# ox-vgg/wise

Hardware: AMD Instinct MI355X
Metric: frames/sec embedded (ViT-B/32 bs=256) + queries/sec over 10M×512 index, 1/2/4/8 MI355X (higher is better)
Workload: dtype bf16; 1 GPU; OpenCLIP ViT-B/32 image tower (encode_image + L2 normalise), bs=256 frames per GPU, fp32 normalised frames resident in HBM -> [256,512] fp32 unit vectors; seeded random weights (no checkpoints offline); batches_in_flight=2, distinct_input_batches=4, layernorm_fold=True, global_batch=256, frames_per_gpu=256, parallelism=dp1, device=AMD Radeon Graphics

## Files before the change

wise_amd/csrc/gemm_bf16.hip:

```cpp
#include <utility>
#include <vector>

#include "common.h"
#include "transformer.h"
#include "gemm_shared.h"
#include "gemm_w4.h"

namespace wise {

struct GemmPlan {
    int splitk = 0;
    int n = 1;
    int v[2] = {0, 0};
    int rows[2] = {0, 0};
};

enum ConvTile { CONV_128x64 = 0, CONV_128x128 = 1, CONV_256x64 = 2, CONV_PP256 = 3 };

static int resolve_variant(int v, int M, int N, int K, int mode) {
    if (v >= 60 && v <= 70) {
        bool ok = false;
        switch (v) {
            case 60: ok = w4_shape_ok(M, N, K, 8); break;
            case 61: ok = w4_shape_ok(M, N, K, 5); break;
// ... 1754 lines not shown
static void launch_fold_consumer(int v, const bf16_t* A, const bf16_t* Wt, const float* bias, int M, int N, int K, bf16_t* out,
                                 const FoldArgs& fa, hipStream_t st) {
    switch (v) {
        case 60: launch_w4<MODE, 8, 8, 3, 2, 1, 1>(A, Wt, bias, M, N, K, out, st, fa); break;
        case 61: launch_w4<MODE, 5, 8, 3, 2, 1, 1>(A, Wt, bias, M, N, K, out, st, fa); break;
        case 64: launch_w4p<MODE, 1>(A, Wt, bias, M, N, K, out, device_cus(), st, fa); break;
        case 68: launch_w4<MODE, 4, 8, 3, 2, 1, 1>(A, Wt, bias, M, N, K, out, st, fa); break;
        case 66: launch_w4<MODE, 8, 6, 3, 2, 1, 1>(A, Wt, bias, M, N, K, out, st, fa); break;
        case 67: launch_w4<MODE, 4, 6, 3, 2, 1, 1>(A, Wt, bias, M, N, K, out, st, fa); break;
        case 69: launch_w4<MODE, 4, 6, 2, 2, 2, 1>(A, Wt, bias, M, N, K, out, st, fa); break;
        default: launch_w4<MODE, 4, 4, 3, 2, 2, 1>(A, Wt, bias, M, N, K, out, st, fa); break;
    }
}

int gemm_fold_bf16(const bf16_t* A, const bf16_t* Wt, const float* bias, const float* rstd, int M, int N, int K, int mode,
                   bf16_t* out, hipStream_t st) {
    WISE_CHECK_ARG(A && Wt && bias && rstd && out, "gemm_fold_bf16: null pointer");
    WISE_CHECK_ARG(gemm_fold_shape_ok(M, N, K) && bf16_out(mode) && mode != EPI_RELU, "gemm_fold_bf16: M=%d N=%d K=%d mode=%d", M, N, K, mode);
    ProfScope prof(PROF_GEMM, 2.0 * (double)M * (double)N * (double)K, st);
    FoldArgs fa;
    fa.stats = const_cast<float*>(rstd);
    const int v = fold_plan(M, N, K, mode, false, false, device_cus());
    WISE_CHECK_ARG(v != 0, "gemm_fold_bf16: no tile for M=%d N=%d K=%d", M, N, K);
    switch (mode) {
        case EPI_BF16: launch_fold_consumer<EPI_BF16>(v, A, Wt, bias, M, N, K, out, fa, st); break;
        case EPI_QUICKGELU: launch_fold_consumer<EPI_QUICKGELU>(v, A, Wt, bias, M, N, K, out, fa, st); break;
        case EPI_GELU: launch_fold_consumer<EPI_GELU>(v, A, Wt, bias, M, N, K, out, fa, st); break;
        default: launch_fold_consumer<EPI_GELU_TANH>(v, A, Wt, bias, M, N, K, out, fa, st); break;
    }
    WISE_LAUNCH_CHECK("gemm_w4_kernel (fold, bf16 out)");
    return WISE_OK;
}

size_t gemm_fold_stats_bytes(int M, int N) { return fold_stats_bytes(M, N); }
size_t gemm_fold_counters_bytes(int M) { return fold_count_slots(M) * 4; }

// ... 133 lines not shown
        const int r[6] = {p.splitk, p.n, p.v[0], p.rows[0], p.v[1], p.rows[1]};
        for (int i = 0; i < 6; ++i) out[i] = r[i];
        return 6;
    }
    if (kind == 1) {
        out[0] = wise::fold_plan(a[0], a[1], a[2], a[3], a[4] != 0, a[5] != 0, a[6]);
        return 1;
    }
    if (kind == 2) {
        out[0] = wise::conv_plan(wise::conv_rows(a[0], a[1], a[2], a[5] != 0), a[4]);
        return 1;
    }
    return 0;
}

extern "C" size_t wise_debug_gemm_splitk_bytes(int M, int m_valid, int N, int K) { return wise::gemm_splitk_bytes(M, m_valid, N, K); }
extern "C" int wise_debug_gemm_rows(const uint16_t* A, const uint16_t* Wt, const float* bias, int M, int m_valid, int N, int K,
                                    int mode, void* out, float* sk, size_t sk_bytes, void* stream) {
    return wise::gemm_bf16_rows(A, Wt, bias, M, m_valid, N, K, mode, out, (hipStream_t)stream, sk, sk_bytes);
}
extern "C" int wise_debug_gemm_resid_ln_rows(const uint16_t* A, const uint16_t* Wt, const float* bias, int M, int m_valid,
                                             int ln_rows, int N, int K, float* x, const float* ln_w, const float* ln_b, float eps,
                                             int post_ln, uint16_t* h, float* sk, size_t sk_bytes, void* stream) {
    return wise::gemm_resid_ln_rows(A, Wt, bias, M, m_valid, ln_rows, N, K, x, ln_w, ln_b, eps, post_ln != 0, h,
                                    (hipStream_t)stream, sk, sk_bytes);
}
#endif
```

wise_amd/csrc/gemm_w4.h:

```cpp
#pragma once
#include <type_traits>
#include "gemm_shared.h"

namespace wise {

struct FoldArgs {
    float* stats = nullptr;
    bf16_t* hcopy = nullptr;
    float eps = 1e-5f;
    int group32 = 0;
    int lo_off = 0;
};
__host__ __device__ inline size_t fold_count_slots(int M) { return (size_t)((M / 128 + 1 + 63) / 64 * 64); }
__host__ __device__ inline size_t fold_stats_bytes(int M, int N) { return (size_t)M * 4 + fold_count_slots(M) * 4 + (size_t)M * (N / 32) * 8; }

namespace w4 {

#ifdef W4_STAMPS
__device__ unsigned long long g_w4p_stamps[4][4];
#define W4P_STAMP(t, k) do { if (threadIdx.x == 0 && blockIdx.x == 0 && (t) < 4) g_w4p_stamps[t][k] = __builtin_amdgcn_s_memtime(); } while (0)
__device__ unsigned long long g_w4_stamps[2][4];
#define W4_STAMP(k)                                                                                              \
    do {                                                                                                         \
        if (threadIdx.x == 0 && (blockIdx.x == 0 || blockIdx.x == gridDim.x - 1))                                \
            g_w4_stamps[blockIdx.x == 0 ? 0 : 1][k] = __builtin_amdgcn_s_memtime();                              \
    } while (0)
// ... 131 lines not shown
        case 21: asm volatile("v_accvgpr_read_b32 %0, a244\n\tv_accvgpr_read_b32 %1, a245\n\tv_accvgpr_read_b32 %2, a246\n\tv_accvgpr_read_b32 %3, a247" : "=v"(r.x), "=v"(r.y), "=v"(r.z), "=v"(r.w) : : W4_HI_AGPRS); break;
        case 22: asm volatile("v_accvgpr_read_b32 %0, a248\n\tv_accvgpr_read_b32 %1, a249\n\tv_accvgpr_read_b32 %2, a250\n\tv_accvgpr_read_b32 %3, a251" : "=v"(r.x), "=v"(r.y), "=v"(r.z), "=v"(r.w) : : W4_HI_AGPRS); break;
        case 23: asm volatile("v_accvgpr_read_b32 %0, a252\n\tv_accvgpr_read_b32 %1, a253\n\tv_accvgpr_read_b32 %2, a254\n\tv_accvgpr_read_b32 %3, a255" : "=v"(r.x), "=v"(r.y), "=v"(r.z), "=v"(r.w) : : W4_HI_AGPRS); break;
        default: break;
    }
    return r;
}

template <int CTRL>
__device__ __forceinline__ float dpp_add(float v) {
    return v + __builtin_bit_cast(float, __builtin_amdgcn_update_dpp(0, __builtin_bit_cast(int, v), CTRL, 0xF, 0xF, true));
}

template <int MODE, int MI, int NJ, int RI, int FOLD = 0>
__device__ __forceinline__ void epi_bf16_pass(const f32x4 (&acc)[MI][NJ], int i0, const float4 (&bv)[NJ], bf16_t* __restrict__ out,
                                              int N, int row0, int col0, int lane, unsigned my,
                                              const float* __restrict__ rstd = nullptr) {
    constexpr int RS = NJ * 32 + 16, CPR = NJ * 2;
    static_assert((RI * 16 * CPR) % 64 == 0, "walk covers the piece in whole wave instructions");
    const int l15 = lane & 15, g = lane >> 4;
    float rs[RI];
    if constexpr (FOLD == 1) {
#pragma unroll
        for (int ii = 0; ii < RI; ++ii) rs[ii] = rstd[row0 + (i0 + ii) * 16 + l15];
    }
#pragma unroll
    for (int j = 0; j < NJ; j += 2)
#pragma unroll
        for (int ii = 0; ii < RI; ++ii) {
            const f32x4 a = acc[i0 + ii][j], b = acc[i0 + ii][j + 1];
            float x[8];
// ... 5 lines not shown
                x[0] = a[0] + bv[j].x; x[1] = a[1] + bv[j].y; x[2] = a[2] + bv[j].z; x[3] = a[3] + bv[j].w;
                x[4] = b[0] + bv[j + 1].x; x[5] = b[1] + bv[j + 1].y; x[6] = b[2] + bv[j + 1].z; x[7] = b[3] + bv[j + 1].w;
            }
            act_apply_n<MODE, 8>(x);
            W4_LDS(u32x2_t, my + (ii * 16 + l15) * RS + (j * 16 + g * 4) * 2) = u32x2_t{pack_bf16x2(x[0], x[1]), pack_bf16x2(x[2], x[3])};
            W4_LDS(u32x2_t, my + (ii * 16 + l15) * RS + ((j + 1) * 16 + g * 4) * 2) = u32x2_t{pack_bf16x2(x[4], x[5]), pack_bf16x2(x[6], x[7])};
        }
    __builtin_amdgcn_fence(__ATOMIC_RELEASE, "wavefront");
    __builtin_amdgcn_wave_barrier();
    __builtin_amdgcn_fence(__ATOMIC_ACQUIRE, "wavefront");
#pragma unroll
    for (int t = 0; t < RI * 16 * CPR / 64; ++t) {
        const int idx = t * 64 + lane, row = idx / CPR, c = idx % CPR;
        const u32x4_t v = W4_LDS(const u32x4_t, my + row * RS + c * 16);
#ifdef W4_PLAIN_STORES
        *reinterpret_cast<u32x4_t*>(out + (size_t)(row0 + i0 * 16 + row) * N + col0 + c * 8) = v;
#else
        __builtin_nontemporal_store(v, reinterpret_cast<u32x4_t*>(out + (size_t)(row0 + i0 * 16 + row) * N + col0 + c * 8));
#endif
    }
    __builtin_amdgcn_fence(__ATOMIC_RELEASE, "wavefront");
    __builtin_amdgcn_wave_barrier();
    __builtin_amdgcn_fence(__ATOMIC_ACQUIRE, "wavefront");
}

template <int NJ, int RI>
__device__ __forceinline__ void resid_load(const float* __restrict__ out, int N, int row0, int col0, int lane,
                                           float4 (&res)[RI * 16 * NJ * 4 / 64]) {
    constexpr int CPR = NJ * 4;
#pragma unroll
    for (int t = 0; t < RI * 16 * CPR / 64; ++t) {
        const int idx = t * 64 + lane, row = idx / CPR, c = idx % CPR;
        res[t] = *reinterpret_cast<const float4*>(out + (size_t)(row0 + row) * N + col0 + c * 4);
// ... 242 lines not shown
    mfma_retire();
#pragma unroll
    for (int m = 0; m < MI * NJ; ++m) { if (m < 64) pin_a(acc[m / NJ][m % NJ]); else pin_v(acc[m / NJ][m % NJ]); }

    W4_STAMP(2);
    asm volatile("s_waitcnt lgkmcnt(0)" ::: "memory");
    __builtin_amdgcn_s_barrier();
    const int row0 = m0 + wm * MI * 16, col0 = n0 + wn * NJ * 16;
    float4 bv[NJ];
#pragma unroll
    for (int j = 0; j < NJ; ++j)
        bv[j] = bias ? *reinterpret_cast<const float4*>(bias + col0 + j * 16 + g * 4) : make_float4(0.f, 0.f, 0.f, 0.f);
    const unsigned my = wave * 20480;
    if constexpr (bf16_out(MODE)) {
        bf16_t* o = reinterpret_cast<bf16_t*>(out);
        if constexpr (MI % 4 != 0) epi_bf16_pass<MODE, MI, NJ, MI % 4, FOLD>(acc, MI - MI % 4, bv, o, N, row0, col0, lane, my, fold.stats);
#pragma unroll
        for (int i0 = (MI / 4 - 1) * 4; i0 >= 0; i0 -= 4) epi_bf16_pass<MODE, MI, NJ, 4, FOLD>(acc, i0, bv, o, N, row0, col0, lane, my, fold.stats);
    } else {
        float* o = reinterpret_cast<float*>(out);
        constexpr int RP = NJ == 8 ? 2 : 1;
        constexpr int NP = (MI + RP - 1) / RP, NRES = RP * 16 * NJ * 4 / 64;
        static_assert(MI % RP == 0 || RP == 2, "passes");
        float4 res[2][NRES];
        auto load = [&](int p, float4 (&r)[NRES]) {
            if (p * RP + RP <= MI) {
                if constexpr (FOLD == 2) resid_load_hilo<NJ, RP>(fold.hcopy, fold.lo_off, N, row0 + p * RP * 16, col0, lane, r);
                else resid_load<NJ, RP>(o, N, row0 + p * RP * 16, col0, lane, r);
            } else if constexpr (RP == 2) {
                float4 (&h)[NRES / 2] = reinterpret_cast<float4 (&)[NRES / 2]>(r);
                if constexpr (FOLD == 2) resid_load_hilo<NJ, 1>(fold.hcopy, fold.lo_off, N, row0 + p * RP * 16, col0, lane, h);
                else resid_load<NJ, 1>(o, N, row0 + p * RP * 16, col0, lane, h);
            }
// ... 129 lines not shown

    f32x4 acc[MI][NJ];
    bf16x8 af0[MI], wf0[NJ], af1[MI], wf1[NJ];
    {
        lds_cptr pw = (lds_cptr)(uintptr_t)fw0, pa = (lds_cptr)(uintptr_t)fa0;
#pragma unroll
        for (int j = 0; j < NJ; ++j) wf0[j] = *reinterpret_cast<const __attribute__((address_space(3))) bf16x8*>(pw + j * 2048);
#pragma unroll
        for (int i = 0; i < MI; ++i) af0[i] = *reinterpret_cast<const __attribute__((address_space(3))) bf16x8*>(pa + i * 2048);
    }
    unsigned oA0 = 0, oA1 = ASZ, oA2 = 2 * ASZ;
    unsigned oW0 = 0, oW1 = WSZ, oW2 = 0;

    u32x2_t packed[MI][NJ];
    const __amdgpu_buffer_rsrc_t rO = __builtin_amdgcn_make_buffer_rsrc((void*)out, 0, 0x7fffffff, 0x00020000);
    const int vst = (g * N + l15 * 8) * 2;
    int sst = 0;
    typedef __attribute__((address_space(3))) unsigned char* lds_ptr;
    const lds_ptr scw = (lds_ptr)(uintptr_t)(scr + l15 * 272 + g * 8);
    const lds_cptr scrd = (lds_cptr)(uintptr_t)(scr + g * 272 + l15 * 16);
    auto load_bias = [&](int ncol, f32x4 (&b)[NJ]) {
#pragma unroll
        for (int j = 0; j < NJ; ++j) {
            const float4 v = bias ? *reinterpret_cast<const float4*>(bias + ncol + wn * 128 + j * 16 + g * 4) : make_float4(0.f, 0.f, 0.f, 0.f);
            b[j] = f32x4{v.x, v.y, v.z, v.w};
        }
    };
    f32x4 bv[NJ];
    float rs[MI];

    auto phase = [&](const bf16x8 (&af)[MI], const bf16x8 (&wf)[NJ], bf16x8 (&afn)[MI], bf16x8 (&wfn)[NJ], lds_cptr pw,
// ... 9 lines not shown
        for (int m = 0; m < NM; ++m) {
            if (m % MPR == 0 && m / MPR < NR) {
                const int r = m / MPR;
                if (r < NJ) wfn[r] = *reinterpret_cast<const __attribute__((address_space(3))) bf16x8*>(pw + r * 2048);
                else afn[r - NJ] = *reinterpret_cast<const __attribute__((address_space(3))) bf16x8*>(pa + (r - NJ) * 2048);
            }
            if (m >= 1 && (m - 1) % MPD == 0 && (m - 1) / MPD < ND) {
                const int u = ((m - 1) / MPD) * 4 + wave;
                dma16(rq, dslot + u * 1024, voff, u * 8 * ldb + dkb);
            }
            if (DW && m % 4 == 3 && m / 4 < NJ)
                *reinterpret_cast<__attribute__((address_space(3))) u32x2_t*>(scw + (m / 4) * 32) = packed[DI][m / 4];
            if (DR && m % 8 == 3 && m / 8 < 4)
                piece[m / 8] = *reinterpret_cast<const __attribute__((address_space(3))) u32x4_t*>(scrd + (m / 8) * 4 * 272);
            if (DR && m % 8 == 1 && m >= 9)
                __builtin_amdgcn_raw_buffer_store_b128(piece[m / 8 - 1], rO, vst, sst + (DI * 16 + (m / 8 - 1) * 4) * N * 2, 2);
            if (INIT) mfma16a_init(acc[m / NJ][m % NJ], wf[m % NJ], af[m / NJ]);
            else mfma16a(acc[m / NJ][m % NJ], wf[m % NJ], af[m / NJ]);
        }
    };

    auto step = [&](auto init_c, auto di_c, __amdgpu_buffer_rsrc_t rqA, __amdgpu_buffer_rsrc_t rqW, int kq) {
        constexpr int DI = decltype(di_c)::value;
        using DIc = std::integral_constant<int, DI < 0 ? 0 : DI>;
        using DOc = std::integral_constant<bool, (DI >= 0)>;
        phase(af0, wf0, af1, wf1, (lds_cptr)(uintptr_t)(oW0 + fw1), (lds_cptr)(uintptr_t)(oA0 + fa1), init_c,
              std::integral_constant<int, PA>{}, rqA, oA2, kq, DIc{}, DOc{}, std::false_type{});
        asm volatile("s_waitcnt lgkmcnt(0)" ::: "memory");
        wait_vmcnt<PA>();
        __builtin_amdgcn_s_barrier();
        phase(af1, wf1, af0, wf0, (lds_cptr)(uintptr_t)(oW1 + fw0), (lds_cptr)(uintptr_t)(oA1 + fa0), std::false_type{},
// ... 40 lines not shown

#pragma unroll
        for (int i = 0; i < MI; ++i)
#pragma unroll
            for (int j = 0; j < NJ; j += 2) {
                float x[8];
#pragma unroll
                for (int r = 0; r < 4; ++r) {
                    if constexpr (FOLD == 1) { x[r] = fmaf(acc[i][j][r], rs[i], bv[j][r]); x[4 + r] = fmaf(acc[i][j + 1][r], rs[i], bv[j + 1][r]); }
                    else { x[r] = acc[i][j][r] + bv[j][r]; x[4 + r] = acc[i][j + 1][r] + bv[j + 1][r]; }
                }
                act_apply_n<MODE, 8>(x);
                packed[i][j] = u32x2_t{pack_bf16x2(x[0], x[1]), pack_bf16x2(x[2], x[3])};
                packed[i][j + 1] = u32x2_t{pack_bf16x2(x[4], x[5]), pack_bf16x2(x[6], x[7])};
            }
        sst = ((m0 + wm * 80) * N + n0 + wn * 128) * 2;
        m0 = m0n; n0 = n0n; rA = rAn; rW = rWn;
        W4P_STAMP(t, 3);
    }
    wait_vmcnt<0>();
#pragma unroll
    for (int i = 0; i < MI; ++i) {
#pragma unroll
        for (int j = 0; j < NJ; ++j) *reinterpret_cast<__attribute__((address_space(3))) u32x2_t*>(scw + j * 32) = packed[i][j];
#pragma unroll
        for (int t4 = 0; t4 < 4; ++t4) {
            const u32x4_t v = *reinterpret_cast<const __attribute__((address_space(3))) u32x4_t*>(scrd + t4 * 4 * 272);
            __builtin_amdgcn_raw_buffer_store_b128(v, rO, vst, sst + (i * 16 + t4 * 4) * N * 2, 2);
        }
    }
}

template <int MODE, int FOLD = 0>
static void launch_w4p(const bf16_t* A, const bf16_t* Wt, const float* bias, int M, int N, int K, void* out, int num_cus,
                       hipStream_t st, const FoldArgs fold = FoldArgs()) {
    if constexpr (bf16_out(MODE)) {
        auto kern = gemm_w4p_kernel<MODE, FOLD>;
        constexpr int LDS = 3 * 160 * 128 + 2 * 256 * 128 + 4 * 16 * 272;
        static PerDeviceOnce attr_set;
        attr_set([&] {
            raise_lds_limit(reinterpret_cast<const void*>(kern), LDS);
        });
        const int ntiles = (M / 160) * (N / 256);
// ... 13 lines not shown
```

wise_amd/csrc/transformer.h:

```cpp
#pragma once
#include "common.h"

namespace wise {

int gemm_bf16(const bf16_t* A, const bf16_t* Wt, const float* bias, int M, int N, int K, int mode, void* out,
              hipStream_t st);
size_t gemm_splitk_bytes(int M, int m_valid, int N, int K);
int gemm_bf16_rows(const bf16_t* A, const bf16_t* Wt, const float* bias, int M, int m_valid, int N, int K, int mode,
                   void* out, hipStream_t st, float* sk = nullptr, size_t sk_bytes = 0);
int conv3x3_bf16(const bf16_t* X, const bf16_t* Wt, const float* bias, const bf16_t* zeros, int B, int T, int F, int Cin,
                 int Cout, bool pool, bf16_t* out, hipStream_t st);
int gemm_resid_ln_rows(const bf16_t* A, const bf16_t* Wt, const float* bias, int M, int m_valid, int ln_rows, int N, int K,
                       float* x, const float* ln_w, const float* ln_b, float eps, bool post_ln, bf16_t* h, hipStream_t st,
                       float* sk = nullptr, size_t sk_bytes = 0);
bool gemm_fold_shape_ok(int M, int N, int K);
int gemm_fold_bf16(const bf16_t* A, const bf16_t* Wt, const float* bias, const float* rstd, int M, int N, int K, int mode,
                   bf16_t* out, hipStream_t st);
size_t gemm_fold_stats_bytes(int M, int N);
int gemm_fold_resid(const bf16_t* A, const bf16_t* Wt, const float* bias, int M, int N, int K, bf16_t* hi, long long lo_off,
                    float* stats, float eps, hipStream_t st, int group32 = 0, bool accumulate = true );
size_t gemm_fold_counters_bytes(int M);
void gemm_set_overlapped(bool on);
int layernorm_f32_bf16(const float* x, const float* w, const float* b, int rows, int W, float eps, bf16_t* y,
                       hipStream_t st);
int attention_bf16(const bf16_t* qkv, int B, int T, int H, bf16_t* o, hipStream_t st, bool causal, int dh = 64,
                   const int* lens = nullptr);
int layernorm_f32_dual(const float* x, const float* w, const float* b, int rows, int W, float eps, float* xo, bf16_t* y,
                       hipStream_t st);

struct BlockWeights {
    const bf16_t* wb; size_t per_layer_b, in_proj, out_proj, c_fc, c_proj;
    const float* pf; size_t per_layer_f, ln1_w, ln1_b, in_b, out_b, ln2_w, ln2_b, fc_b, proj_b;
// ... 35 lines not shown
```

wise_amd/csrc/vit.hip:

```cpp
#include "transformer.h"
#include "gemm_w4.h"

namespace wise {
#ifdef WISE_DEBUG_KNOBS
static int g_ablate = 0;
#else
constexpr int g_ablate = 0;
#endif

template <int NV>
__global__ __launch_bounds__(256) void layernorm_kernel(const float* x , const float* __restrict__ w,
                                                        const float* __restrict__ b, int rows, int W, float eps,
                                                        bf16_t* __restrict__ y, float* xo = nullptr) {
    const int lane = threadIdx.x & 63;
    const int row = blockIdx.x * 4 + (threadIdx.x >> 6);
    if (row >= rows) return;
    const int w4 = W >> 2;
    const float4* xr = reinterpret_cast<const float4*>(x + (size_t)row * W);
    float4 v[NV];
    float s = 0.f;
#pragma unroll
    for (int i = 0; i < NV; ++i) {
        const int c = i * 64 + lane;
        v[i] = (c < w4) ? xr[c] : make_float4(0.f, 0.f, 0.f, 0.f);
// ... 225 lines not shown
            }
            pf[ks][qt] = f;
        }
    }
}

struct ClsRows {
    const bf16_t* hi = nullptr;
    long long lo_off = 0;
    bf16_t* hc = nullptr;
    long long lc_off = 0;
    const float* rs = nullptr;
    float* rs_c = nullptr;
    int* cnt = nullptr;
    int ncnt = 0;
};
__device__ __forceinline__ void cls_row_copy(const ClsRows& cr, int b, int T, int W, int lane) {
    const uint2* src = reinterpret_cast<const uint2*>(cr.hi + (size_t)b * T * W);
    uint2* dst = reinterpret_cast<uint2*>(cr.hc + (size_t)b * W);
    const long long so = cr.lo_off >> 2, dof = cr.lc_off >> 2;
    for (int c = lane; c < (W >> 2); c += 64) {
        dst[c] = src[c];
        dst[c + dof] = src[c + so];
    }
    if (cr.rs && lane == 0) cr.rs_c[b] = cr.rs[(size_t)b * T];
    if (b == 0)
        for (int c = lane; c < cr.ncnt; c += 64) cr.cnt[c] = 0;
}

template <int QT, bool CAUSAL, int DH = 64, bool PF = false, bool CLS = false>
// ... 11 lines not shown
    const int qc = (int)(item % nqc);
    const int h = (int)((item / nqc) % H);
    const int b = (int)(item / ((long long)nqc * H));
    const int W = H * DH, W3 = 3 * W;
    const bf16_t* base = qkv + (size_t)b * T * W3;
    unsigned char* vimg = v_all[wave];
    const int l15 = lane & 15, g = lane >> 4;
    const int Tk = lens ? max(1, min(T, lens[b])) : T;

    const bf16x8 zero8 = {0, 0, 0, 0, 0, 0, 0, 0};
    bf16x8 qf[QT][NS];
#pragma unroll
    for (int qt = 0; qt < QT; ++qt) {
        int t = CLS ? 0 : qc * (16 * QT) + qt * 16 + l15;
        if (t >= T) t = T - 1;
#pragma unroll
        for (int s = 0; s < NS; ++s)
            qf[qt][s] = (s * 32 + g * 8 < DH) ? *reinterpret_cast<const bf16x8*>(base + (size_t)t * W3 + h * DH + s * 32 + g * 8)
                                              : zero8;
    }

    f32x4 oacc[ND][QT];
#pragma unroll
    for (int i = 0; i < ND; ++i)
#pragma unroll
        for (int j = 0; j < QT; ++j) oacc[i][j] = f32x4{0.f, 0.f, 0.f, 0.f};
    float mrun[QT], lrun[QT];
#pragma unroll
    for (int qt = 0; qt < QT; ++qt) { mrun[qt] = -INFINITY; lrun[qt] = 0.f; }

    const int q_last = min(T, (qc + 1) * (16 * QT)) - 1;
    const int nkb = CAUSAL ? (q_last >> 6) + 1 : (Tk + 63) >> 6;
    constexpr int CPR = DH / 8;
    auto load_k = [&](int kb, bf16x8 (&kf)[4][NS]) {
// ... 145 lines not shown
        }
    }
    if constexpr (CLS) {
        if (h == 0 && cr.hi) cls_row_copy(cr, b, T, W, lane);
    }
}

__global__ __launch_bounds__(256) void cls_rows_kernel(int B, int T, int W, const ClsRows cr) {
    const int b = blockIdx.x * 4 + (threadIdx.x >> 6);
    if (b < B) cls_row_copy(cr, b, T, W, threadIdx.x & 63);
}

static int g_attn_qt = 0;

int attention_cls(const bf16_t* qkv, int B, int T, int H, int W, bf16_t* o, const ClsRows& cr, hipStream_t st) {
    WISE_CHECK_ARG(qkv && o && B > 0 && T > 0 && H > 0 && (!cr.hi || (cr.hc && (!cr.rs || cr.rs_c) && (!cr.ncnt || cr.cnt))),
                   "attention_cls: bad argument");
    WISE_CHECK_ARG(W == H * 64, "attention_cls: head dim 64 only (W=%d, H=%d)", W, H);
    const long long items = (long long)B * H;
    hipLaunchKernelGGL((attention_kernel<1, false, 64, false, true>), dim3((unsigned)((items + 3) / 4)), dim3(256), 0, st, qkv, B, T, H, o,
                       (const int*)nullptr, cr);
    WISE_LAUNCH_CHECK("attention_kernel (class query)");
    return WISE_OK;
}

int attention_bf16(const bf16_t* qkv, int B, int T, int H, bf16_t* o, hipStream_t st, bool causal, int dh, const int* lens) {
    WISE_CHECK_ARG(qkv && o && B > 0 && T > 0 && H > 0, "attention: bad argument");
    WISE_CHECK_ARG(dh == 64 || (dh == 80 && !causal), "attention: head dim %d (64, or 80 without a mask)", dh);
    WISE_CHECK_ARG(!lens || (dh == 64 && !causal), "attention: per-sequence key counts go with head dim 64 and no causal mask");
    if (g_ablate & 4) return WISE_OK;
    if (dh == 80) {
// ... 437 lines not shown
    const float inv = 1.f / ps;
    float mine = 0.f;
#pragma unroll
    for (int j = 0; j < 64; ++j) {
        const float tot = wave_sum(acc[j]);
        if (lane == j) mine = tot * inv;
    }
    o[(size_t)b * W + h * 64 + lane] = f32_to_bf16(mine);
}

template <int NV>
__global__ __launch_bounds__(256) void embed_lnpre_kernel(const float* __restrict__ patch_out,
                                                          const float* __restrict__ cls, const float* __restrict__ pos,
                                                          const float* __restrict__ w, const float* __restrict__ bb,
                                                          int rows, int T, int W, float eps, float* __restrict__ x,
                                                          bf16_t* __restrict__ hcopy, float* __restrict__ rstd_out, long long lo_off) {
    const int lane = threadIdx.x & 63;
    const int row = blockIdx.x * 4 + (threadIdx.x >> 6);
    if (row >= rows) return;
    const int b = row / T, t = row % T;
    const int w4 = W >> 2;
    const float4* src = (t == 0) ? reinterpret_cast<const float4*>(cls)
                                 : reinterpret_cast<const float4*>(patch_out + ((size_t)b * (T - 1) + (t - 1)) * W);
    const float4* pr = reinterpret_cast<const float4*>(pos + (size_t)t * W);
    float4 v[NV];
    float s = 0.f;
#pragma unroll
    for (int i = 0; i < NV; ++i) {
        const int c = i * 64 + lane;
        if (c < w4) {
            float4 a = src[c], p = pr[c];
            v[i] = make_float4(a.x + p.x, a.y + p.y, a.z + p.z, a.w + p.w);
        } else
            v[i] = make_float4(0.f, 0.f, 0.f, 0.f);
// ... 132 lines not shown
                                     false, h, st, sk, sk_bytes)))
            return rc;
        if ((rc = gemm_bf16_rows(h, lwb + bw.c_fc, lpf + bw.fc_b, Mp, Mv, F, W, act == 0 ? 1 : (act == 1 ? 2 : 5), a, st, sk, sk_bytes))) return rc;
        if (l + 1 < L) {
            const float* npf = bw.pf + bw.per_layer_f * (l + 1);
            if ((rc = gemm_resid_ln_rows(a, lwb + bw.c_proj, lpf + bw.proj_b, Mp, Mv, M, W, F, x, npf + bw.ln1_w, npf + bw.ln1_b, eps,
                                         false, h, st, sk, sk_bytes)))
                return rc;
        } else if ((rc = gemm_bf16_rows(a, lwb + bw.c_proj, lpf + bw.proj_b, Mp, Mv, W, F, 3, x, st, sk, sk_bytes))) {
            return rc;
        }
    }
    return WISE_OK;
}

struct ClsTail {
    bf16_t* hc;
    bf16_t* o;
    float* stats;
    bf16_t* hb;
    int Bp;
};
static int transformer_blocks_fold(const BlockWeights& bw, int L, int W, int H, int F, int act, int batch, int T, float* x,
                                   bf16_t* h, bf16_t* qkv, bf16_t* a, float* stats, hipStream_t st, float eps, bool fuse_attn,
                                   const ClsTail* tail) {
    const int M = batch * T, Mp = (M + 255) / 256 * 256;
    int rc;
    float* rstd = stats;
    if (hipMemsetAsync(stats + Mp, 0, gemm_fold_counters_bytes(Mp), st) != hipSuccess) {
        set_error("vit_forward: memset of the fold counters failed");
        return WISE_E_INVALID;
    }
    bf16_t* hi = reinterpret_cast<bf16_t*>(x);
    const long long lo_off = (long long)Mp * W;
    bf16_t* ao = h;
    for (int l = 0; l < L; ++l) {
        const bf16_t* lwb = bw.wb + bw.per_layer_b * l;
        const float* lpf = bw.pf + bw.per_layer_f * l;
        if ((rc = gemm_fold_bf16(hi, lwb + bw.in_proj, lpf + bw.in_b, rstd, Mp, 3 * W, W, 0, qkv, st))) return rc;
        if (tail && l == L - 1) {
            const int Bp = tail->Bp;
            const long long lc_off = (long long)Bp * W;
            ClsRows cr;
            cr.hi = hi; cr.lo_off = lo_off; cr.hc = tail->hc; cr.lc_off = lc_off;
            cr.cnt = reinterpret_cast<int*>(tail->stats + Bp); cr.ncnt = (int)(gemm_fold_counters_bytes(Bp) / 4);
            if (fuse_attn) {
                if ((rc = attention_oproj_fold(qkv, batch, T, H, lwb + bw.out_proj, lpf + bw.out_b, hi, lo_off, rstd, eps, st))) return rc;
                cr.rs = rstd; cr.rs_c = tail->stats;
                hipLaunchKernelGGL(cls_rows_kernel, dim3((unsigned)((batch + 3) / 4)), dim3(256), 0, st, batch, T, W, cr);
                WISE_LAUNCH_CHECK("cls_rows_kernel");
            } else {
                if ((rc = attention_cls(qkv, batch, T, H, W, tail->o, cr, st))) return rc;
                if ((rc = gemm_fold_resid(tail->o, lwb + bw.out_proj, lpf + bw.out_b, Bp, W, W, tail->hc, lc_off, tail->stats, eps, st))) return rc;
            }
            if ((rc = gemm_fold_bf16(tail->hc, lwb + bw.c_fc, lpf + bw.fc_b, tail->stats, Bp, F, W, act == 0 ? 1 : (act == 1 ? 2 : 5), tail->o, st)))
                return rc;
            if ((rc = gemm_fold_resid(tail->o, lwb + bw.c_proj, lpf + bw.proj_b, Bp, W, F, tail->hc, lc_off, tail->stats, eps, st))) return rc;
            break;
        }
        if (fuse_attn) {
            if ((rc = attention_oproj_fold(qkv, batch, T, H, lwb + bw.out_proj, lpf + bw.out_b, hi, lo_off, rstd, eps, st))) return rc;
// ... 105 lines not shown
    size_t off = 0;
    w.x = off; off += align_up((size_t)w.Mp * d.W * 4, 256);
    w.h = off; off += align_up((size_t)w.Mp * d.W * 2, 256);
    size_t qkv_b = (size_t)w.Mp * 3 * d.W * 2, po_b = (size_t)w.Mpp * d.W * 4;
    w.qkv = off; off += align_up(qkv_b > po_b ? qkv_b : po_b, 256);
    size_t a_b = (size_t)w.Mp * d.F * 2, pa_b = (size_t)w.Mpp * d.Kp * 2;
    const size_t head_b = (size_t)((B + 255) / 256 * 256) * (d.W + d.F) * 2;
    if (pa_b > a_b) a_b = pa_b;
    if (d.arch == 1 && head_b > a_b) a_b = head_b;
    w.a = off; off += align_up(a_b, 256);
    w.rstd = off; off += align_up(gemm_fold_stats_bytes(w.Mp, d.W), 256);
    w.total = off;
    return w;
}

#ifdef WISE_DEBUG_KNOBS
static int g_cls_tail = 1;
#else
constexpr int g_cls_tail = 1;
#endif

static bool cls_tail_layout(const VitDims& d, const VitWs& ws, int batch, unsigned char* wsb, ClsTail* t) {
    if (!d.fold || d.arch != 0 || !g_cls_tail || d.W != d.H * 64) return false;
    const size_t W = d.W, F = d.F, Bp = (size_t)(batch + 127) / 128 * 128, Bh = (size_t)(batch + 255) / 256 * 256;
    const size_t oa = align_up(Bp * std::max(W, F) * 2, 256), e_b = align_up(Bh * d.D * 4, 256);
    if (2 * Bp * W * 2 > ws.qkv - ws.h || oa + gemm_fold_stats_bytes((int)Bp, d.W) > ws.rstd - ws.a || (size_t)batch * W * 4 > ws.rstd - ws.a ||
        e_b + Bh * W * 2 > ws.a - ws.qkv)
        return false;
    t->hc = reinterpret_cast<bf16_t*>(wsb + ws.h);
    t->o = reinterpret_cast<bf16_t*>(wsb + ws.a);
    t->stats = reinterpret_cast<float*>(wsb + ws.a + oa);
    t->hb = reinterpret_cast<bf16_t*>(wsb + ws.qkv + e_b);
    t->Bp = (int)Bp;
    return true;
}

template <int NV>
static void launch_embed(const float* po, const float* cls, const float* pos, const float* w, const float* b, int rows,
                         int T, int W, float* x, hipStream_t st, bf16_t* hcopy, float* rstd_out, long long lo_off) {
    hipLaunchKernelGGL(embed_lnpre_kernel<NV>, dim3((rows + 3) / 4), dim3(256), 0, st, po, cls, pos, w, b, rows, T, W,
                       1e-5f, x, hcopy, rstd_out, lo_off);
}

__global__ __launch_bounds__(256) void hilo_rows_kernel(const bf16_t* __restrict__ hi, long long lo_off, int n, int stride, int W,
                                                        float* __restrict__ out, int ostride) {
    const long long i = (long long)blockIdx.x * 256 + threadIdx.x;
    if (i >= (long long)n * W) return;
    const int r = (int)(i / W), c = (int)(i % W);
    const size_t src = (size_t)r * stride * W + c;
    out[(size_t)r * ostride * W + c] = bf16_to_f32(hi[src]) + bf16_to_f32(hi[src + lo_off]);
}

static int vit_forward_part(const wise_vit_config* cfg, const VitDims& d, const VitOffsets& o, const bf16_t* wb,
                            const float* pf, const void* images, int in_kind, int batch, float* out,
                            unsigned char* wsb, hipStream_t st) {
    const VitWs ws = vit_ws(d, batch);
// ... 25 lines not shown
                           reinterpret_cast<const float*>(images), batch, d.S, d.P, d.g, d.Kp, patches, nc);
    WISE_LAUNCH_CHECK("patchify_kernel");
    rc = gemm_bf16(patches, wb + o.conv1, nullptr, ws.Mpp, W, d.Kp, 4, patch_out, st);
    if (rc) return rc;
    if (d.arch == 1) {
        const long long total4 = (long long)ws.M * (W >> 2);
        hipLaunchKernelGGL(embed_pos_kernel, dim3((unsigned)((total4 + 255) / 256)), dim3(256), 0, st, patch_out, pf + o.pos,
                           total4, d.T, W, x);
        WISE_LAUNCH_CHECK("embed_pos_kernel");
    } else {

        const int nv = (W / 4 + 63) / 64;
        bf16_t* fh = d.fold ? reinterpret_cast<bf16_t*>(x) : nullptr;
        float* frs = d.fold ? reinterpret_cast<float*>(wsb + ws.rstd) : nullptr;
        const long long flo = (long long)ws.Mp * W;
        const float* cls = pf + o.cls; const float* pos = pf + o.pos;
        const float* lw = pf + o.ln_pre_w; const float* lb = pf + o.ln_pre_b;
        switch (nv) {
            case 1: launch_embed<1>(patch_out, cls, pos, lw, lb, ws.M, d.T, W, x, st, fh, frs, flo); break;
            case 2: launch_embed<2>(patch_out, cls, pos, lw, lb, ws.M, d.T, W, x, st, fh, frs, flo); break;
            case 3: launch_embed<3>(patch_out, cls, pos, lw, lb, ws.M, d.T, W, x, st, fh, frs, flo); break;
            case 4: launch_embed<4>(patch_out, cls, pos, lw, lb, ws.M, d.T, W, x, st, fh, frs, flo); break;
            case 5: launch_embed<5>(patch_out, cls, pos, lw, lb, ws.M, d.T, W, x, st, fh, frs, flo); break;
            case 6: launch_embed<6>(patch_out, cls, pos, lw, lb, ws.M, d.T, W, x, st, fh, frs, flo); break;
            case 7: launch_embed<7>(patch_out, cls, pos, lw, lb, ws.M, d.T, W, x, st, fh, frs, flo); break;
            case 8: launch_embed<8>(patch_out, cls, pos, lw, lb, ws.M, d.T, W, x, st, fh, frs, flo); break;
            default: set_error("vit_forward: width %d too large", W); return WISE_E_UNSUPPORTED;
        }
        WISE_LAUNCH_CHECK("embed_lnpre_kernel");
    }
    const BlockWeights bw = {wb + o.layer0_b, o.per_layer_b, o.in_proj, o.out_proj, o.c_fc, o.c_proj,
                             pf + o.layer0_f, o.per_layer_f, o.ln1_w, o.ln1_b, o.in_b, o.out_b, o.ln2_w, o.ln2_b,
                             o.fc_b, o.proj_b};
    ClsTail tail;
    const bool cls_tail = cls_tail_layout(d, ws, batch, wsb, &tail);
    if (d.fold) {
        if ((rc = transformer_blocks_fold(bw, d.L, W, d.H, d.F, cfg->act, batch, d.T, x, h, qkv, a,
                                          reinterpret_cast<float*>(wsb + ws.rstd), st, 1e-5f, d.fold == 2, cls_tail ? &tail : nullptr)))
            return rc;
    } else if ((rc = transformer_blocks(bw, d.L, W, d.H, d.F, cfg->act, batch, d.T, false, x, h, qkv, a, st,
                                        d.arch == 1 ? 1e-6f : 1e-5f)))
// ... 216 lines not shown
    return WISE_OK;
}

extern "C" int wise_layernorm_f32_bf16(const float* x, const float* w, const float* b, int rows, int W, float eps,
                                       uint16_t* y, void* stream) {
    return layernorm_f32_bf16(x, w, b, rows, W, eps, y, (hipStream_t)stream);
}

extern "C" int wise_attention_bf16(const uint16_t* qkv, int B, int T, int H, uint16_t* o, void* stream) {
    return attention_bf16(qkv, B, T, H, o, (hipStream_t)stream, false, 64);
}

#ifdef WISE_DEBUG_KNOBS
extern "C" int wise_debug_set_gemm_flags(int flags) { wise::g_ablate = flags & 6; return 0; }
extern "C" int wise_debug_set_vit_cls_tail(int on) { wise::g_cls_tail = on ? 1 : 0; return 0; }
extern "C" int wise_debug_attention_cls_bf16(const uint16_t* qkv, int B, int T, int H, uint16_t* o, void* stream) {
    return wise::attention_cls(qkv, B, T, H, H * 64, o, wise::ClsRows(), (hipStream_t)stream);
}
extern "C" int wise_debug_ao_set(int flags) { wise::g_ao_dbg = flags & 15; return 0; }
extern "C" int wise_debug_ao_stamps(unsigned long long* out) {
    return hipMemcpyFromSymbol(out, HIP_SYMBOL(wise::g_ao_stamps), sizeof(unsigned long long) * 96) == hipSuccess ? 0 : -1;
}
#endif
extern "C" int wise_attention_oproj_fold(const uint16_t* qkv, int B, int T, int H, const uint16_t* Wt, const float* bias,
                                         uint16_t* hi, int64_t lo_off, float* rstd, float eps, void* stream) {
    WISE_CHECK_ARG(lo_off >= (int64_t)B * T * H * 64, "attention_oproj_fold: lo_off %lld overlaps the hi rows", (long long)lo_off);
    return attention_oproj_fold(qkv, B, T, H, Wt, bias, hi, (long long)lo_off, rstd, eps, (hipStream_t)stream);
}

extern "C" int wise_attention_dh_bf16(const uint16_t* qkv, int B, int T, int H, int dh, uint16_t* o, void* stream) {
// ... 10 lines not shown
```

Baseline: 106,400 frames/s.

## Compute last-layer Q only for CLS rows and fold counter reset into embed

```diff
diff --git a/wise_amd/csrc/gemm_bf16.hip b/wise_amd/csrc/gemm_bf16.hip
--- a/wise_amd/csrc/gemm_bf16.hip
+++ b/wise_amd/csrc/gemm_bf16.hip
@@ -1792,12 +1792,15 @@
 }
 
 int gemm_fold_bf16(const bf16_t* A, const bf16_t* Wt, const float* bias, const float* rstd, int M, int N, int K, int mode,
-                   bf16_t* out, hipStream_t st) {
+                   bf16_t* out, hipStream_t st, int ldo) {
     WISE_CHECK_ARG(A && Wt && bias && rstd && out, "gemm_fold_bf16: null pointer");
     WISE_CHECK_ARG(gemm_fold_shape_ok(M, N, K) && bf16_out(mode) && mode != EPI_RELU, "gemm_fold_bf16: M=%d N=%d K=%d mode=%d", M, N, K, mode);
+    WISE_CHECK_ARG(ldo == 0 || (ldo >= N && ldo % 8 == 0 && ((uintptr_t)out & 15) == 0 && (long long)M * ldo * 2 < 0x7fffffffLL),
+                   "gemm_fold_bf16: output row stride %d (N=%d, M=%d)", ldo, N, M);
     ProfScope prof(PROF_GEMM, 2.0 * (double)M * (double)N * (double)K, st);
     FoldArgs fa;
     fa.stats = const_cast<float*>(rstd);
+    fa.ldo = ldo == N ? 0 : ldo;
     const int v = fold_plan(M, N, K, mode, false, false, device_cus());
     WISE_CHECK_ARG(v != 0, "gemm_fold_bf16: no tile for M=%d N=%d K=%d", M, N, K);
     switch (mode) {
@@ -1961,6 +1964,11 @@
     return 0;
 }
 
+extern "C" int wise_debug_gemm_fold_bf16_ld(const uint16_t* A, const uint16_t* Wt, const float* bias, const float* rstd, int M, int N,
+                                            int K, int mode, uint16_t* out, int ldo, void* stream) {
+    return wise::gemm_fold_bf16(A, Wt, bias, rstd, M, N, K, mode, out, (hipStream_t)stream, ldo);
+}
+
 extern "C" size_t wise_debug_gemm_splitk_bytes(int M, int m_valid, int N, int K) { return wise::gemm_splitk_bytes(M, m_valid, N, K); }
 extern "C" int wise_debug_gemm_rows(const uint16_t* A, const uint16_t* Wt, const float* bias, int M, int m_valid, int N, int K,
                                     int mode, void* out, float* sk, size_t sk_bytes, void* stream) {
diff --git a/wise_amd/csrc/gemm_w4.h b/wise_amd/csrc/gemm_w4.h
--- a/wise_amd/csrc/gemm_w4.h
+++ b/wise_amd/csrc/gemm_w4.h
@@ -10,6 +10,7 @@
     float eps = 1e-5f;
     int group32 = 0;
     int lo_off = 0;
+    int ldo = 0;
 };
 __host__ __device__ inline size_t fold_count_slots(int M) { return (size_t)((M / 128 + 1 + 63) / 64 * 64); }
 __host__ __device__ inline size_t fold_stats_bytes(int M, int N) { return (size_t)M * 4 + fold_count_slots(M) * 4 + (size_t)M * (N / 32) * 8; }
@@ -171,7 +172,7 @@
 
 template <int MODE, int MI, int NJ, int RI, int FOLD = 0>
 __device__ __forceinline__ void epi_bf16_pass(const f32x4 (&acc)[MI][NJ], int i0, const float4 (&bv)[NJ], bf16_t* __restrict__ out,
-                                              int N, int row0, int col0, int lane, unsigned my,
+                                              int ldo, int row0, int col0, int lane, unsigned my,
                                               const float* __restrict__ rstd = nullptr) {
     constexpr int RS = NJ * 32 + 16, CPR = NJ * 2;
     static_assert((RI * 16 * CPR) % 64 == 0, "walk covers the piece in whole wave instructions");
@@ -207,9 +208,9 @@
         const int idx = t * 64 + lane, row = idx / CPR, c = idx % CPR;
         const u32x4_t v = W4_LDS(const u32x4_t, my + row * RS + c * 16);
 #ifdef W4_PLAIN_STORES
-        *reinterpret_cast<u32x4_t*>(out + (size_t)(row0 + i0 * 16 + row) * N + col0 + c * 8) = v;
+        *reinterpret_cast<u32x4_t*>(out + (size_t)(row0 + i0 * 16 + row) * ldo + col0 + c * 8) = v;
 #else
-        __builtin_nontemporal_store(v, reinterpret_cast<u32x4_t*>(out + (size_t)(row0 + i0 * 16 + row) * N + col0 + c * 8));
+        __builtin_nontemporal_store(v, reinterpret_cast<u32x4_t*>(out + (size_t)(row0 + i0 * 16 + row) * ldo + col0 + c * 8));
 #endif
     }
     __builtin_amdgcn_fence(__ATOMIC_RELEASE, "wavefront");
@@ -482,9 +483,10 @@
     const unsigned my = wave * 20480;
     if constexpr (bf16_out(MODE)) {
         bf16_t* o = reinterpret_cast<bf16_t*>(out);
-        if constexpr (MI % 4 != 0) epi_bf16_pass<MODE, MI, NJ, MI % 4, FOLD>(acc, MI - MI % 4, bv, o, N, row0, col0, lane, my, fold.stats);
-#pragma unroll
-        for (int i0 = (MI / 4 - 1) * 4; i0 >= 0; i0 -= 4) epi_bf16_pass<MODE, MI, NJ, 4, FOLD>(acc, i0, bv, o, N, row0, col0, lane, my, fold.stats);
+        const int ldo = (FOLD == 1 && fold.ldo) ? fold.ldo : N;
+        if constexpr (MI % 4 != 0) epi_bf16_pass<MODE, MI, NJ, MI % 4, FOLD>(acc, MI - MI % 4, bv, o, ldo, row0, col0, lane, my, fold.stats);
+#pragma unroll
+        for (int i0 = (MI / 4 - 1) * 4; i0 >= 0; i0 -= 4) epi_bf16_pass<MODE, MI, NJ, 4, FOLD>(acc, i0, bv, o, ldo, row0, col0, lane, my, fold.stats);
     } else {
         float* o = reinterpret_cast<float*>(out);
         constexpr int RP = NJ == 8 ? 2 : 1;
@@ -644,7 +646,8 @@
 
     u32x2_t packed[MI][NJ];
     const __amdgpu_buffer_rsrc_t rO = __builtin_amdgcn_make_buffer_rsrc((void*)out, 0, 0x7fffffff, 0x00020000);
-    const int vst = (g * N + l15 * 8) * 2;
+    const int ldo = (FOLD == 1 && fold.ldo) ? fold.ldo : N;
+    const int vst = (g * ldo + l15 * 8) * 2;
     int sst = 0;
     typedef __attribute__((address_space(3))) unsigned char* lds_ptr;
     const lds_ptr scw = (lds_ptr)(uintptr_t)(scr + l15 * 272 + g * 8);
@@ -684,7 +687,7 @@
             if (DR && m % 8 == 3 && m / 8 < 4)
                 piece[m / 8] = *reinterpret_cast<const __attribute__((address_space(3))) u32x4_t*>(scrd + (m / 8) * 4 * 272);
             if (DR && m % 8 == 1 && m >= 9)
-                __builtin_amdgcn_raw_buffer_store_b128(piece[m / 8 - 1], rO, vst, sst + (DI * 16 + (m / 8 - 1) * 4) * N * 2, 2);
+                __builtin_amdgcn_raw_buffer_store_b128(piece[m / 8 - 1], rO, vst, sst + (DI * 16 + (m / 8 - 1) * 4) * ldo * 2, 2);
             if (INIT) mfma16a_init(acc[m / NJ][m % NJ], wf[m % NJ], af[m / NJ]);
             else mfma16a(acc[m / NJ][m % NJ], wf[m % NJ], af[m / NJ]);
         }
@@ -755,7 +758,7 @@
                 packed[i][j] = u32x2_t{pack_bf16x2(x[0], x[1]), pack_bf16x2(x[2], x[3])};
                 packed[i][j + 1] = u32x2_t{pack_bf16x2(x[4], x[5]), pack_bf16x2(x[6], x[7])};
             }
-        sst = ((m0 + wm * 80) * N + n0 + wn * 128) * 2;
+        sst = ((m0 + wm * 80) * ldo + n0 + wn * 128) * 2;
         m0 = m0n; n0 = n0n; rA = rAn; rW = rWn;
         W4P_STAMP(t, 3);
     }
@@ -767,7 +770,7 @@
 #pragma unroll
         for (int t4 = 0; t4 < 4; ++t4) {
             const u32x4_t v = *reinterpret_cast<const __attribute__((address_space(3))) u32x4_t*>(scrd + t4 * 4 * 272);
-            __builtin_amdgcn_raw_buffer_store_b128(v, rO, vst, sst + (i * 16 + t4 * 4) * N * 2, 2);
+            __builtin_amdgcn_raw_buffer_store_b128(v, rO, vst, sst + (i * 16 + t4 * 4) * ldo * 2, 2);
         }
     }
 }
diff --git a/wise_amd/csrc/transformer.h b/wise_amd/csrc/transformer.h
--- a/wise_amd/csrc/transformer.h
+++ b/wise_amd/csrc/transformer.h
@@ -15,7 +15,7 @@
                        float* sk = nullptr, size_t sk_bytes = 0);
 bool gemm_fold_shape_ok(int M, int N, int K);
 int gemm_fold_bf16(const bf16_t* A, const bf16_t* Wt, const float* bias, const float* rstd, int M, int N, int K, int mode,
-                   bf16_t* out, hipStream_t st);
+                   bf16_t* out, hipStream_t st, int ldo = 0 );
 size_t gemm_fold_stats_bytes(int M, int N);
 int gemm_fold_resid(const bf16_t* A, const bf16_t* Wt, const float* bias, int M, int N, int K, bf16_t* hi, long long lo_off,
                     float* stats, float eps, hipStream_t st, int group32 = 0, bool accumulate = true );
diff --git a/wise_amd/csrc/vit.hip b/wise_amd/csrc/vit.hip
--- a/wise_amd/csrc/vit.hip
+++ b/wise_amd/csrc/vit.hip
@@ -263,6 +263,8 @@
     float* rs_c = nullptr;
     int* cnt = nullptr;
     int ncnt = 0;
+    const bf16_t* q = nullptr;
+    int q_ld = 0;
 };
 __device__ __forceinline__ void cls_row_copy(const ClsRows& cr, int b, int T, int W, int lane) {
     const uint2* src = reinterpret_cast<const uint2*>(cr.hi + (size_t)b * T * W);
@@ -304,10 +306,13 @@
     for (int qt = 0; qt < QT; ++qt) {
         int t = CLS ? 0 : qc * (16 * QT) + qt * 16 + l15;
         if (t >= T) t = T - 1;
+        const bf16_t* qrow = base + (size_t)t * W3;
+        if constexpr (CLS) {
+            if (cr.q) qrow = cr.q + (size_t)b * cr.q_ld;
+        }
 #pragma unroll
         for (int s = 0; s < NS; ++s)
-            qf[qt][s] = (s * 32 + g * 8 < DH) ? *reinterpret_cast<const bf16x8*>(base + (size_t)t * W3 + h * DH + s * 32 + g * 8)
-                                              : zero8;
+            qf[qt][s] = (s * 32 + g * 8 < DH) ? *reinterpret_cast<const bf16x8*>(qrow + h * DH + s * 32 + g * 8) : zero8;
     }
 
     f32x4 oacc[ND][QT];
@@ -483,7 +488,8 @@
 static int g_attn_qt = 0;
 
 int attention_cls(const bf16_t* qkv, int B, int T, int H, int W, bf16_t* o, const ClsRows& cr, hipStream_t st) {
-    WISE_CHECK_ARG(qkv && o && B > 0 && T > 0 && H > 0 && (!cr.hi || (cr.hc && (!cr.rs || cr.rs_c) && (!cr.ncnt || cr.cnt))),
+    WISE_CHECK_ARG(qkv && o && B > 0 && T > 0 && H > 0 && (!cr.hi || (cr.hc && (!cr.rs || cr.rs_c) && (!cr.ncnt || cr.cnt))) &&
+                       (!cr.q || (cr.q_ld >= W && cr.q_ld % 8 == 0)),
                    "attention_cls: bad argument");
     WISE_CHECK_ARG(W == H * 64, "attention_cls: head dim 64 only (W=%d, H=%d)", W, H);
     const long long items = (long long)B * H;
@@ -951,10 +957,13 @@
                                                           const float* __restrict__ cls, const float* __restrict__ pos,
                                                           const float* __restrict__ w, const float* __restrict__ bb,
                                                           int rows, int T, int W, float eps, float* __restrict__ x,
-                                                          bf16_t* __restrict__ hcopy, float* __restrict__ rstd_out, long long lo_off) {
+                                                          bf16_t* __restrict__ hcopy, float* __restrict__ rstd_out, long long lo_off,
+                                                          int* __restrict__ cnt, int ncnt) {
     const int lane = threadIdx.x & 63;
     const int row = blockIdx.x * 4 + (threadIdx.x >> 6);
     if (row >= rows) return;
+    if (row == 0)
+        for (int c = lane; c < ncnt; c += 64) cnt[c] = 0;
     const int b = row / T, t = row % T;
     const int w4 = W >> 2;
     const float4* src = (t == 0) ? reinterpret_cast<const float4*>(cls)
@@ -1117,6 +1126,12 @@
     return WISE_OK;
 }
 
+#ifdef WISE_DEBUG_KNOBS
+static int g_cls_tail = 1, g_tail_qkv = 1;
+#else
+constexpr int g_cls_tail = 1, g_tail_qkv = 1;
+#endif
+
 struct ClsTail {
     bf16_t* hc;
     bf16_t* o;
@@ -1130,24 +1145,31 @@
     const int M = batch * T, Mp = (M + 255) / 256 * 256;
     int rc;
     float* rstd = stats;
-    if (hipMemsetAsync(stats + Mp, 0, gemm_fold_counters_bytes(Mp), st) != hipSuccess) {
-        set_error("vit_forward: memset of the fold counters failed");
-        return WISE_E_INVALID;
-    }
     bf16_t* hi = reinterpret_cast<bf16_t*>(x);
     const long long lo_off = (long long)Mp * W;
     bf16_t* ao = h;
     for (int l = 0; l < L; ++l) {
         const bf16_t* lwb = bw.wb + bw.per_layer_b * l;
         const float* lpf = bw.pf + bw.per_layer_f * l;
-        if ((rc = gemm_fold_bf16(hi, lwb + bw.in_proj, lpf + bw.in_b, rstd, Mp, 3 * W, W, 0, qkv, st))) return rc;
+        const bool tail_q = tail && l == L - 1 && !fuse_attn && g_tail_qkv && tail->Bp <= Mp;
+        if (!tail_q && (rc = gemm_fold_bf16(hi, lwb + bw.in_proj, lpf + bw.in_b, rstd, Mp, 3 * W, W, 0, qkv, st))) return rc;
         if (tail && l == L - 1) {
             const int Bp = tail->Bp;
             const long long lc_off = (long long)Bp * W;
             ClsRows cr;
             cr.hi = hi; cr.lo_off = lo_off; cr.hc = tail->hc; cr.lc_off = lc_off;
             cr.cnt = reinterpret_cast<int*>(tail->stats + Bp); cr.ncnt = (int)(gemm_fold_counters_bytes(Bp) / 4);
-            if (fuse_attn) {
+            if (tail_q) {
+                cr.rs = rstd; cr.rs_c = tail->stats;
+                hipLaunchKernelGGL(cls_rows_kernel, dim3((unsigned)((batch + 3) / 4)), dim3(256), 0, st, batch, T, W, cr);
+                WISE_LAUNCH_CHECK("cls_rows_kernel");
+                if ((rc = gemm_fold_bf16(hi, lwb + bw.in_proj + (size_t)W * W, lpf + bw.in_b + W, rstd, Mp, 2 * W, W, 0, qkv + W, st, 3 * W))) return rc;
+                if ((rc = gemm_fold_bf16(tail->hc, lwb + bw.in_proj, lpf + bw.in_b, tail->stats, Bp, W, W, 0, qkv, st, 3 * W))) return rc;
+                ClsRows cq;
+                cq.q = qkv; cq.q_ld = 3 * W;
+                if ((rc = attention_cls(qkv, batch, T, H, W, tail->o, cq, st))) return rc;
+                if ((rc = gemm_fold_resid(tail->o, lwb + bw.out_proj, lpf + bw.out_b, Bp, W, W, tail->hc, lc_off, tail->stats, eps, st))) return rc;
+            } else if (fuse_attn) {
                 if ((rc = attention_oproj_fold(qkv, batch, T, H, lwb + bw.out_proj, lpf + bw.out_b, hi, lo_off, rstd, eps, st))) return rc;
                 cr.rs = rstd; cr.rs_c = tail->stats;
                 hipLaunchKernelGGL(cls_rows_kernel, dim3((unsigned)((batch + 3) / 4)), dim3(256), 0, st, batch, T, W, cr);
@@ -1283,11 +1305,6 @@
     return w;
 }
 
-#ifdef WISE_DEBUG_KNOBS
-static int g_cls_tail = 1;
-#else
-constexpr int g_cls_tail = 1;
-#endif
 
 static bool cls_tail_layout(const VitDims& d, const VitWs& ws, int batch, unsigned char* wsb, ClsTail* t) {
     if (!d.fold || d.arch != 0 || !g_cls_tail || d.W != d.H * 64) return false;
@@ -1306,9 +1323,9 @@
 
 template <int NV>
 static void launch_embed(const float* po, const float* cls, const float* pos, const float* w, const float* b, int rows,
-                         int T, int W, float* x, hipStream_t st, bf16_t* hcopy, float* rstd_out, long long lo_off) {
+                         int T, int W, float* x, hipStream_t st, bf16_t* hcopy, float* rstd_out, long long lo_off, int* cnt, int ncnt) {
     hipLaunchKernelGGL(embed_lnpre_kernel<NV>, dim3((rows + 3) / 4), dim3(256), 0, st, po, cls, pos, w, b, rows, T, W,
-                       1e-5f, x, hcopy, rstd_out, lo_off);
+                       1e-5f, x, hcopy, rstd_out, lo_off, cnt, ncnt);
 }
 
 __global__ __launch_bounds__(256) void hilo_rows_kernel(const bf16_t* __restrict__ hi, long long lo_off, int n, int stride, int W,
@@ -1364,17 +1381,19 @@
         bf16_t* fh = d.fold ? reinterpret_cast<bf16_t*>(x) : nullptr;
         float* frs = d.fold ? reinterpret_cast<float*>(wsb + ws.rstd) : nullptr;
         const long long flo = (long long)ws.Mp * W;
+        int* fcnt = d.fold ? reinterpret_cast<int*>(frs + ws.Mp) : nullptr;
+        const int nfcnt = d.fold ? (int)(gemm_fold_counters_bytes(ws.Mp) / 4) : 0;
         const float* cls = pf + o.cls; const float* pos = pf + o.pos;
         const float* lw = pf + o.ln_pre_w; const float* lb = pf + o.ln_pre_b;
         switch (nv) {
-            case 1: launch_embed<1>(patch_out, cls, pos, lw, lb, ws.M, d.T, W, x, st, fh, frs, flo); break;
-            case 2: launch_embed<2>(patch_out, cls, pos, lw, lb, ws.M, d.T, W, x, st, fh, frs, flo); break;
-            case 3: launch_embed<3>(patch_out, cls, pos, lw, lb, ws.M, d.T, W, x, st, fh, frs, flo); break;
-            case 4: launch_embed<4>(patch_out, cls, pos, lw, lb, ws.M, d.T, W, x, st, fh, frs, flo); break;
-            case 5: launch_embed<5>(patch_out, cls, pos, lw, lb, ws.M, d.T, W, x, st, fh, frs, flo); break;
-            case 6: launch_embed<6>(patch_out, cls, pos, lw, lb, ws.M, d.T, W, x, st, fh, frs, flo); break;
-            case 7: launch_embed<7>(patch_out, cls, pos, lw, lb, ws.M, d.T, W, x, st, fh, frs, flo); break;
-            case 8: launch_embed<8>(patch_out, cls, pos, lw, lb, ws.M, d.T, W, x, st, fh, frs, flo); break;
+            case 1: launch_embed<1>(patch_out, cls, pos, lw, lb, ws.M, d.T, W, x, st, fh, frs, flo, fcnt, nfcnt); break;
+            case 2: launch_embed<2>(patch_out, cls, pos, lw, lb, ws.M, d.T, W, x, st, fh, frs, flo, fcnt, nfcnt); break;
+            case 3: launch_embed<3>(patch_out, cls, pos, lw, lb, ws.M, d.T, W, x, st, fh, frs, flo, fcnt, nfcnt); break;
+            case 4: launch_embed<4>(patch_out, cls, pos, lw, lb, ws.M, d.T, W, x, st, fh, frs, flo, fcnt, nfcnt); break;
+            case 5: launch_embed<5>(patch_out, cls, pos, lw, lb, ws.M, d.T, W, x, st, fh, frs, flo, fcnt, nfcnt); break;
+            case 6: launch_embed<6>(patch_out, cls, pos, lw, lb, ws.M, d.T, W, x, st, fh, frs, flo, fcnt, nfcnt); break;
+            case 7: launch_embed<7>(patch_out, cls, pos, lw, lb, ws.M, d.T, W, x, st, fh, frs, flo, fcnt, nfcnt); break;
+            case 8: launch_embed<8>(patch_out, cls, pos, lw, lb, ws.M, d.T, W, x, st, fh, frs, flo, fcnt, nfcnt); break;
             default: set_error("vit_forward: width %d too large", W); return WISE_E_UNSUPPORTED;
         }
         WISE_LAUNCH_CHECK("embed_lnpre_kernel");
@@ -1621,6 +1640,7 @@
 #ifdef WISE_DEBUG_KNOBS
 extern "C" int wise_debug_set_gemm_flags(int flags) { wise::g_ablate = flags & 6; return 0; }
 extern "C" int wise_debug_set_vit_cls_tail(int on) { wise::g_cls_tail = on ? 1 : 0; return 0; }
+extern "C" int wise_debug_set_vit_tail_qkv(int on) { wise::g_tail_qkv = on ? 1 : 0; return 0; }
 extern "C" int wise_debug_attention_cls_bf16(const uint16_t* qkv, int B, int T, int H, uint16_t* o, void* stream) {
     return wise::attention_cls(qkv, B, T, H, H * 64, o, wise::ClsRows(), (hipStream_t)stream);
 }
```

Result: no change. 106,500 frames/s (median of 2 runs) (+0.1%).
